# DLR-RM/curvature

Hardware: AMD Instinct MI355X
Metric: KFAC factor-build + invert + sample throughput (higher is better)
Workload: dtype f32

## Files before the change

### curvature_amd/csrc/invert.hip

```cpp
#include <type_traits>
#include "kernarg.h"
#include "mma64.h"
#include <hip/hip_ext.h>

#include <algorithm>
#include <chrono>
#include <cstdlib>
#include <mutex>
#include <vector>

namespace curv {

constexpr int INV_THREADS = MMA_THREADS;
constexpr int SQ_FLAGS = 32;
constexpr int SQ_FD = 0, SQ_FLC = 4, SQ_FLROW = 8, SQ_FT = 12;
constexpr int SQ_SPIN_LIMIT = 1 << 21;
#ifdef CURV_SQ_TRACE
__device__ long long g_sq_trace[256];
#define KT_BEGIN(slot) { if (threadIdx.x == 0 && k0 == 4 * (CURV_SQ_TRACE - 1)) atomicMax((unsigned long long*)&g_sq_trace[slot], (1ull << 62) - (unsigned long long)wall_clock64()); }
#define KT_END(slot) { if (threadIdx.x == 0 && k0 == 4 * (CURV_SQ_TRACE - 1)) atomicMax((unsigned long long*)&g_sq_trace[slot], (unsigned long long)wall_clock64()); }
#define SQT(slot) { if (threadIdx.x == 0 && f == 0 && stamp == CURV_SQ_TRACE) g_sq_trace[slot] = wall_clock64(); }
#define FIT(k) { if (threadIdx.x == 0 && trace_base >= 0) g_sq_trace[trace_base + (k)] = wall_clock64(); }
#else
#define SQT(slot)
#define FIT(k)
#define KT_BEGIN(slot) {}
#define KT_END(slot) {}
#endif
#ifdef CURV_SQ_TRACE
#define PQT(slot) { if (threadIdx.x == 0 && blockIdx.x == 0 && k0 == 4 * (CURV_SQ_TRACE - 1)) g_sq_trace[slot] = wall_clock64(); }
#else
#define PQT(slot)
#endif

struct InvDev {
  const float* F;
  float* L;
  double* W;
  double* X;
  int* info;
  int n, np, P;
  float sqrt_s, sqrt_n;
  int reverse;
  int f64_in;
  int r_minus;
  double* Xout;
  const double* R;
  double* Zm;
  double add64;
  float* C32;
  float* X32;
  float* S32;
  double pivot_min;
};
typedef __attribute__((address_space(1))) float gfloat;
__device__ __host__ __forceinline__ bool s_in_sweep(const InvDev& d) { return d.X32 == nullptr; }
__device__ __host__ __forceinline__ int s_kind(const InvDev& d) { return d.X32 != nullptr ? 0 : (d.Zm != nullptr ? 2 : 1); }

template <typename CountFn>
__device__ __forceinline__ bool locate(const InvDev* __restrict__ t, int nf, int bid, CountFn cnt, int& f,
                                       int& local) {
  const int lane = threadIdx.x & 63;
  int base = 0;
  for (int f0 = 0; f0 < nf; f0 += 64) {
    const int ff = f0 + lane;
    const int c = (ff < nf) ? cnt(t[ff]) : 0;
    int incl = c;
#pragma unroll
    for (int o = 1; o < 64; o <<= 1) {
      const int v = __shfl_up(incl, o, 64);
      if (lane >= o) incl += v;
    }
    const int total = __builtin_amdgcn_readfirstlane(__shfl(incl, 63, 64));
    if (bid < base + total) {
      const unsigned long long m = __ballot(bid < base + incl);
      const int l = __ffsll((long long)m) - 1;
      f = __builtin_amdgcn_readfirstlane(f0 + l);
      local = __builtin_amdgcn_readfirstlane(bid - (base + __shfl(incl - c, l, 64)));
      return true;
    }
    base += total;
  }
  return false;
}

__global__ void __launch_bounds__(INV_THREADS)
inv_prepare_kernel(const InvDev* __restrict__ t, int nf, int* __restrict__ flags) {
  int f, tile;
  if (!locate(t, nf, blockIdx.x, [](const InvDev& d) { return d.P * (d.P + 1) / 2; }, f, tile)) return;
  const InvDev& d = t[f];
  int bi = 0;
  while (tile > bi) { tile -= bi + 1; ++bi; }
  const int bj = tile;
  const int n = d.n, np = d.np, rev = d.reverse;
  const float ss = d.sqrt_s, sn = d.sqrt_n;
  const gfloat* F = (const gfloat*)d.F;
  gdouble* W = (gdouble*)d.W;
  if (bi == 0 && bj == 0 && threadIdx.x == 0) *d.info = 0;
  if (bi == 0 && bj == 0 && threadIdx.x < SQ_FLAGS) flags[(long long)f * SQ_FLAGS + threadIdx.x] = 0;
  if (d.Zm != nullptr) {
    const gdouble* Rg = (const gdouble*)d.R;
    gdouble* Z = (gdouble*)d.Zm;
    const int w0 = __builtin_amdgcn_readfirstlane(threadIdx.x >> 6), c0 = threadIdx.x & 63;
    const int jj = bj * NB + c0;
#pragma unroll 4
    for (int u = 0; u < 16; ++u) {
      const int i = bi * NB + w0 + 4 * u;
      Z[(long long)i * np + jj] = (i < n && jj <= i) ? Rg[(long long)i * n + jj] : 0.0;
    }
  }
  if (d.f64_in) {
    const gdouble* M = (const gdouble*)d.F;
    const int w0 = __builtin_amdgcn_readfirstlane(threadIdx.x >> 6), c0 = threadIdx.x & 63;
    const int jj = bj * NB + c0;
#pragma unroll 4
    for (int u = 0; u < 16; ++u) {
      const int i = bi * NB + w0 + 4 * u;
      double v;
      if (i < n && jj < n) {
        v = 0.5 * (M[(long long)i * n + jj] + M[(long long)jj * n + i]);
        if (i == jj) v += d.add64;
      } else {
        v = (i == jj) ? 1.0 : 0.0;
      }
      W[(long long)i * np + jj] = v;
    }
    return;
  }
  __shared__ float Tm[NB][NB + 1];
  const int w = __builtin_amdgcn_readfirstlane(threadIdx.x >> 6), c = threadIdx.x & 63;
  const int j = bj * NB + c, rj = rev ? n - 1 - j : j;
  const int mi = bi * NB + c, rmi = rev ? n - 1 - mi : mi;
  float fd[16], fm[16];
#pragma unroll
  for (int u = 0; u < 16; ++u) {
    const int r = w + 4 * u;
    const int i = bi * NB + r, ri = rev ? n - 1 - i : i;
    const int mj = bj * NB + r, rmj = rev ? n - 1 - mj : mj;
    fd[u] = (i < n && j < n) ? F[(long long)ri * n + rj] : 0.0f;
    fm[u] = (mi < n && mj < n) ? F[(long long)rmj * n + rmi] : 0.0f;
  }
#pragma unroll
  for (int u = 0; u < 16; ++u) Tm[w + 4 * u][c] = fm[u];
  __syncthreads();
#pragma unroll
  for (int u = 0; u < 16; ++u) {
    const int r = w + 4 * u;
    const int i = bi * NB + r;
    double v;
    if (i < n && j < n) {
      float a = __fmul_rn(ss, fd[u]);
      float b = __fmul_rn(ss, Tm[c][r]);
      if (i == j) { a = __fadd_rn(a, sn); b = __fadd_rn(b, sn); }
      v = (double)__fmul_rn(__fadd_rn(a, b), 0.5f);
    } else {
      v = (i == j) ? 1.0 : 0.0;
    }
    W[(long long)i * np + j] = v;
  }
}

__device__ __host__ __forceinline__ long long inner_tiles(int P, int k, int k0, int kend) {
  const int ke = kend < P ? kend : P;
  long long tr = 0;
  for (int j = k + 1; j < ke; ++j) tr += ke - j;
  const long long sr = (ke - k - 1 > 0) ? (long long)(ke - k - 1) * (k - k0 + 1) : 0;
  return tr + sr;
}
constexpr int SB = 4;
__device__ __host__ __forceinline__ long long outer_tiles(int P, int kend, int row0, bool s_part) {
  const long long r = P - row0;
  if (r <= 0) return 0;
  const long long nsb = (r + SB - 1) / SB, ncb = s_part ? (kend + SB - 1) / SB : 0;
  return (nsb * (nsb + 1) / 2 + nsb * ncb) * (SB * SB);
}
__device__ __host__ __forceinline__ long long strip_tiles(int P, int kend, int lo, int hi, bool s_part) {
  const int re = hi < P ? hi : P;
  long long n = 0;
  for (int j = lo; j < re; ++j) n += P - j;
  if (s_part && re > lo) n += (long long)(re - lo) * kend;
  return n;
}

__device__ __forceinline__ void store_sub(gdouble* C, int np, const f64x4 (&acc)[2][2], int wm, int wn, int lane,
                                          int mode) {
  store_acc(C, np, acc, wm, wn, lane, mode);
}

__device__ __forceinline__ void factor_invert_64(double* Ds, double* Is, int* bad, int pivot_base, double pivot_min, int trace_base = -1);
__device__ __forceinline__ void lds_sub_acc(double* s, const f64x4 (&acc)[2][2], int wm, int wn, int lane);

__global__ void __launch_bounds__(INV_THREADS)
inner_update_kernel(const InvDev* __restrict__ t, int nf, int k, int k0, int kend) {
  __shared__ double As[NB * LDA], Bs[NB * LDA];
  int f, local;
  if (!locate(t, nf, blockIdx.x, [k, k0, kend](const InvDev& d) { return (int)inner_tiles(d.P, k, k0, kend); }, f, local)) return;
  const InvDev& d = t[f];
  const int np = d.np, P = d.P, ke = kend < P ? kend : P;
  gdouble* W = (gdouble*)d.W;
  gdouble* X = (gdouble*)d.X;
  const int lane = threadIdx.x & 63, wave = threadIdx.x >> 6, wm = wave >> 1, wn = wave & 1;
  f64x4 acc[2][2] = {};
  int j = k + 1;
  bool trailing = false;
  for (; j < ke; ++j) {
    if (local < ke - j) { trailing = true; break; }
    local -= ke - j;
  }
  if (trailing) {
    const int i = j + local;
    load_block(W + (long long)i * NB * np + k * NB, np, As);
    if (i != j) load_block(W + (long long)j * NB * np + k * NB, np, Bs);
    __syncthreads();
    mma_64<true>(As, (i != j) ? Bs : As, wm, wn, lane, acc);
    if (i == j && j == k + 1) {
      __shared__ int bad;
      __syncthreads();
      if (threadIdx.x == 0) bad = 0;
      load_block(W + (long long)j * NB * np + j * NB, np, As);
      __syncthreads();
      {
        const int c16 = lane & 15, rq = lane >> 4;
#pragma unroll
        for (int m = 0; m < 2; ++m)
#pragma unroll
          for (int n = 0; n < 2; ++n)
#pragma unroll
            for (int q = 0; q < 4; ++q)
              As[(32 * wm + 16 * m + rq + 4 * q) * LDA + 32 * wn + 16 * n + c16] -= acc[m][n][q];
      }
      __syncthreads();
      factor_invert_64(As, Bs, &bad, j * NB, d.pivot_min);
      store_block(X + (long long)j * NB * np + j * NB, np, Bs);
      if (threadIdx.x == 0 && bad != 0) atomicCAS(d.info, 0, bad);
    } else {
      store_sub(W + (long long)i * NB * np + j * NB, np, acc, wm, wn, lane, 0);
    }
  } else {
    const int w = k - k0 + 1;
    const int a = local / w, jj = k0 + local - a * w;
    const int i = k + 1 + a;
// ... 102 lines not shown
    for (int q = 0; q < 4; ++q) {
      const double v = acc[0][0][q];
      const double out = o.mode == 0 ? old[q] - v : o.mode == 1 ? v : o.mode == 2 ? old[q] + v : -v;
      *(gdouble*)(base + (long long)(4 * q) * np * 8 + voff) = out;
    }
  }
}

template <int WV>
__device__ __forceinline__ void tile_product_k32(const TileJob& o, double* __restrict__ As, double* __restrict__ Bs) {
  if (!o.bt) tile_product_impl<WV, 2>(o, As, Bs);
  else if (o.same) tile_product_impl<WV, 1>(o, As, Bs);
  else tile_product_impl<WV, 0>(o, As, Bs);
}

template <int WV>
__device__ __forceinline__ void outer_update_body(const InvDev* __restrict__ t, int nf, int k0, int kend, int lo, int hi,
                                                  int strip, int n_items, double* __restrict__ As, double* __restrict__ Bs) {
  bool trailing;
  int i, j, f, local;
  if (strip == 1) {
    if (!locate(t, nf, blockIdx.x, [kend, lo, hi](const InvDev& d) { return (int)strip_tiles(d.P, kend, lo, hi, s_in_sweep(d)); }, f, local))
      return;
    const int P = t[f].P, re = hi < P ? hi : P;
    trailing = false;
    j = lo;
    for (; j < re; ++j) {
      if (local < P - j) { trailing = true; break; }
      local -= P - j;
    }
    if (trailing) {
      i = j + local;
    } else {
      const int a = local / kend;
      i = lo + a; j = local - a * kend;
    }
  } else {
    const int row0 = lo;
    int item;
    {
      const int bid = blockIdx.x, xcd = bid & 7, jj = bid >> 3;
      item = ((jj / (SB * SB)) * 8 + xcd) * (SB * SB) + (jj % (SB * SB));
    }
    if (item >= n_items) return;
    if (!locate(t, nf, item, [kend, row0](const InvDev& d) {
          return (int)(outer_tiles(d.P, kend, row0, s_in_sweep(d)) - outer_tiles(d.P, kend, row0, false)); }, f, local)) return;
    const int r = t[f].P - row0;
    const int s2 = local / (SB * SB), in = local % (SB * SB);
    const int di = in / SB, dj = in - di * SB;
    const int ncb = (kend + SB - 1) / SB;
    const int a = s2 / ncb, cb = s2 - a * ncb;
    const int ri = a * SB + di; j = cb * SB + dj;
    if (ri >= r || j >= kend) return;
    trailing = false; i = row0 + ri;
  }
  const InvDev& d = t[f];
  const int np = d.np;
  const gdouble* W = (const gdouble*)d.W;
  gdouble* X = (gdouble*)d.X;
  TileJob o;
  o.np = np;
  o.bt = trailing;
  o.same = trailing && i == j;
  o.a0 = (const gbyte*)(W + (long long)i * NB * np);
  gdouble* Sx = d.Zm != nullptr ? (gdouble*)d.Zm : X;
  o.b0 = trailing ? (const gbyte*)(W + (long long)j * NB * np) : (const gbyte*)(Sx + j * NB);
  o.ke0 = (trailing ? k0 : (j > k0 ? j : k0)) * NB;
  o.ke1 = kend * NB;
  o.C = trailing ? (gdouble*)d.W + (long long)i * NB * np + j * NB : Sx + (long long)i * NB * np + j * NB;
  o.mode = trailing ? 0 : (d.Zm != nullptr ? 0 : (j >= k0 ? 1 : 2));
  tile_product_k32<WV>(o, As, Bs);
}
__global__ void __launch_bounds__(INV_THREADS, 3)
outer_update_kernel(const InvDev* __restrict__ t, int nf, int k0, int kend, int lo, int hi, int strip, int n_items) {
  __shared__ double As[NB * OPA], Bs[NB * OPA > OKS * LDA ? NB * OPA : OKS * LDA];
  outer_update_body<2>(t, nf, k0, kend, lo, hi, strip, n_items, As, Bs);
}
typedef __attribute__((address_space(3))) void lds_void;
typedef __attribute__((address_space(3))) char lds_char;
typedef double f64x2 __attribute__((ext_vector_type(2)));
namespace fard {
constexpr int ROW_B = 128, TILE_B = NB * ROW_B, KS = 16;
}
__global__ void __launch_bounds__(INV_THREADS, 4)
outer_update_dma_kernel(const InvDev* __restrict__ t, int nf, int k0, int kend, int row0, int n_items) {
  using namespace fard;
  __shared__ __attribute__((aligned(1024))) char smem[4 * TILE_B];
  lds_char* lds = (lds_char*)smem;
  int item;
  {
    const int bid = blockIdx.x, xcd = bid & 7, jj = bid >> 3;
    item = ((jj / (SB * SB)) * 8 + xcd) * (SB * SB) + (jj % (SB * SB));
  }
  if (item >= n_items) return;
  int f, local;
  if (!locate(t, nf, item, [kend, row0](const InvDev& d) { return (int)outer_tiles(d.P, kend, row0, false); }, f, local)) return;
  const InvDev& d = t[f];
  int i, j;
  {
    const int r = d.P - row0;
    const int sb = local / (SB * SB), in = local - sb * (SB * SB);
    const int di = in / SB, dj = in - di * SB;
    int a = 0, tl = sb;
    while (tl > a) { tl -= a + 1; ++a; }
    const int ri = a * SB + di, rj = tl * SB + dj;
    if (ri >= r || rj > ri) return;
    i = row0 + ri; j = row0 + rj;
  }
  const int np = d.np;
  const int tid = threadIdx.x, lane = tid & 63;
  const int wave = __builtin_amdgcn_readfirstlane(tid >> 6), wm = wave >> 1, wn = wave & 1;
  const int r16 = lane & 15, kq = lane >> 4;
  const bool same = i == j;
  const unsigned panel_b = (unsigned)((long long)NB * np * 8);
  const __amdgpu_buffer_rsrc_t rs_a =
      __builtin_amdgcn_make_buffer_rsrc((void*)(d.W + (long long)i * NB * np), 0, panel_b, 0x00020000);
  const __amdgpu_buffer_rsrc_t rs_b =
      __builtin_amdgcn_make_buffer_rsrc((void*)(d.W + (long long)j * NB * np), 0, panel_b, 0x00020000);
  const int drow = 8 * wave + (lane >> 3);
  const int voff = (drow * np) * 8 + (((lane & 7) ^ ((drow >> 1) & 7)) << 4);
  const int half_b = 32 * np * 8;
  auto issue = [&](int ke, unsigned buf) {
    const int kb = ke * 8;
    __builtin_amdgcn_raw_ptr_buffer_load_lds(rs_a, (lds_void*)(lds + buf + wave * 1024), 16, voff, kb, 0, 0);
    __builtin_amdgcn_raw_ptr_buffer_load_lds(rs_a, (lds_void*)(lds + buf + (wave + 4) * 1024), 16, voff, half_b + kb, 0, 0);
    if (!same) {
      __builtin_amdgcn_raw_ptr_buffer_load_lds(rs_b, (lds_void*)(lds + 2 * TILE_B + buf + wave * 1024), 16, voff, kb, 0, 0);
      __builtin_amdgcn_raw_ptr_buffer_load_lds(rs_b, (lds_void*)(lds + 2 * TILE_B + buf + (wave + 4) * 1024), 16, voff, half_b + kb, 0, 0);
    }
  };
  unsigned addr_a[2], addr_b[2];
#pragma unroll
  for (int m = 0; m < 2; ++m) {
    const int ra = 32 * wm + 16 * m + r16, rb = 32 * wn + 16 * m + r16;
    addr_a[m] = ra * ROW_B + ((kq ^ ((ra >> 1) & 7)) << 4);
    addr_b[m] = (same ? 0 : 2 * TILE_B) + rb * ROW_B + ((kq ^ ((rb >> 1) & 7)) << 4);
  }
  f64x4 acc[2][2] = {};
  const int ke0 = k0 * NB, n_st = (kend - k0) * NB / KS;
  issue(ke0, 0);
  for (int st = 0; st < n_st; ++st) {
    __builtin_amdgcn_s_waitcnt(0x0f70);
    __syncthreads();
    const unsigned buf = (st & 1) * TILE_B;
    if (st + 1 < n_st) issue(ke0 + KS * (st + 1), TILE_B - buf);
    f64x2 av[2][2], bv[2][2];
#pragma unroll
    for (int h = 0; h < 2; ++h)
#pragma unroll
      for (int m = 0; m < 2; ++m) {
        av[m][h] = *reinterpret_cast<const __attribute__((address_space(3))) f64x2*>(lds + buf + (addr_a[m] ^ (h << 6)));
        bv[m][h] = *reinterpret_cast<const __attribute__((address_space(3))) f64x2*>(lds + buf + (addr_b[m] ^ (h << 6)));
      }
#pragma unroll
    for (int h = 0; h < 2; ++h)
#pragma unroll
      for (int dd = 0; dd < 2; ++dd)
#pragma unroll
        for (int m = 0; m < 2; ++m)
#pragma unroll
          for (int n = 0; n < 2; ++n) acc[m][n] = __builtin_amdgcn_mfma_f64_16x16x4f64(av[m][h][dd], bv[n][h][dd], acc[m][n], 0, 0, 0);
  }
  store_acc((gdouble*)d.W + (long long)i * NB * np + j * NB, np, acc, wm, wn, lane, 0);
}

__global__ void __launch_bounds__(1024)
outer_update_wide_kernel(const InvDev* __restrict__ t, int nf, int k0, int kend, int lo, int hi, int strip, int n_items) {
  __shared__ double As[NB * OPA], Bs[NB * OPA > OKS * LDA ? NB * OPA : OKS * LDA];
  KT_BEGIN(252)
  outer_update_body<4>(t, nf, k0, kend, lo, hi, strip, n_items, As, Bs);
  KT_END(253)
}

__device__ __forceinline__ double readlane_f64(double v, int src_lane) {
  const int lo = __builtin_amdgcn_readlane(__double2loint(v), src_lane);
  const int hi = __builtin_amdgcn_readlane(__double2hiint(v), src_lane);
  return __hiloint2double(hi, lo);
}

template <bool BT>
__device__ __forceinline__ void mma16(const double* Ap, int lda, const double* Bp, int ldb, int lane, f64x4& acc) {
  const int r16 = lane & 15, kq = lane >> 4;
#pragma unroll
  for (int ks = 0; ks < 4; ++ks) {
    const int kk = 4 * ks + kq;
    const double a = Ap[r16 * lda + kk];
    const double b = BT ? Bp[r16 * ldb + kk] : Bp[kk * ldb + r16];
    acc = __builtin_amdgcn_mfma_f64_16x16x4f64(a, b, acc, 0, 0, 0);
  }
}

__device__ __forceinline__ double rsqrt_pos(double x) {
  double y = __builtin_amdgcn_rsq(x);
  const double hx = 0.5 * x;
  y = y * fma(-hx * y, y, 1.5);
  y = y * fma(-hx * y, y, 1.5);
  return y;
}

__device__ __forceinline__ double rcp_pos(double x) {
  const double y = __builtin_amdgcn_rcp(x);
  const double e = fma(-x, y, 1.0);
  return fma(y, fma(e, e, e), y);
}

__device__ __forceinline__ void factor_invert_64(double* Ds, double* Is, int* bad, int pivot_base, double pivot_min, int trace_base) {
  (void)trace_base;
  __shared__ double Sc[4][16 * 17];
  __shared__ double dinv_s[NB];
  const int tid = threadIdx.x, lane = tid & 63, wave = tid >> 6;
  const int r16 = lane & 15, kq = lane >> 4;
  auto diag_inverse = [&](int b) {
    if (lane < 16) {
      const double* Lb = Ds + 16 * b * LDA + 16 * b;
      double x[16], sum[16], col[16], dv[16];
#pragma unroll
      for (int r = 0; r < 16; ++r) { sum[r] = 0.0; col[r] = r > 0 ? Lb[r * LDA] : 0.0; dv[r] = dinv_s[16 * b + r]; }
#pragma unroll
      for (int q = 0; q < 16; ++q) {
        x[q] = ((q == lane ? 1.0 : 0.0) - sum[q]) * dv[q];
        double nxt[16];
#pragma unroll
        for (int r = q + 2; r < 16; ++r) nxt[r] = Lb[r * LDA + q + 1];
#pragma unroll
        for (int r = q + 1; r < 16; ++r) sum[r] += col[r] * x[q];
#pragma unroll
        for (int r = q + 2; r < 16; ++r) col[r] = nxt[r];
      }
#pragma unroll
      for (int r = 0; r < 16; ++r) Is[(16 * b + r) * LDA + 16 * b + lane] = x[r];
    }
  };
  auto wave_sync = [&]() {
    __builtin_amdgcn_fence(__ATOMIC_RELEASE, "wavefront");
    __builtin_amdgcn_wave_barrier();
    __builtin_amdgcn_fence(__ATOMIC_ACQUIRE, "wavefront");
  };
  auto block_sum = [&](int i, int b, int k_lo, int k_hi, f64x4& acc) {
    for (int kk = k_lo; kk < k_hi; ++kk)
      mma16<false>(Ds + 16 * i * LDA + 16 * kk, LDA, Is + 16 * kk * LDA + 16 * b, LDA, lane, acc);
  };
  auto finish_block = [&](int i, int b, const f64x4& acc) {
#pragma unroll
    for (int r = 0; r < 4; ++r) Sc[wave][(kq + 4 * r) * 17 + r16] = acc[r];
// ... 464 lines not shown
  int cf = c, kf = kb;
  fetch(cf, kf, rt0); next(cf, kf);
  if (cf >= 0) { fetch(cf, kf, rt1); next(cf, kf); }
  if (cf >= 0) { fetch(cf, kf, rt2); next(cf, kf); }
  f64x4 acc[4] = {};
  PQT(241)
  [[maybe_unused]] int pq_n = 0;
  auto step = [&](double (&rt)[16]) __attribute__((always_inline)) {
    __syncthreads();
#pragma unroll
    for (int u = 0; u < 16; ++u) Ts[((tid >> 6) + 4 * u) * LDA + (tid & 63)] = rt[u];
    __syncthreads();
    if (cf >= 0) { fetch(cf, kf, rt); next(cf, kf); }
#pragma unroll
    for (int ks = 0; ks < NB / 4; ++ks) {
      const int k = 4 * ks + kq;
      const double a = below ? Own[r16 * PQ_PITCH + 64 * kb + k] : Ts[(16 * wave + r16) * LDA + k];
      const double b = below ? Ts[(16 * wave + r16) * LDA + k] : Own[(64 * kb + k) * 17 + r16];
      acc[ks & 3] = __builtin_amdgcn_mfma_f64_16x16x4f64(a, b, acc[ks & 3], 0, 0, 0);
    }
    if (kb == c) {
      const int wm = below ? q : wave, wn = below ? wave : q;
      const int c16 = lane & 15, rq = lane >> 4;
      gbyte* base = below ? (gbyte*)d.W + (((long long)i * NB) * np + (long long)(k0 + c) * NB) * 8
                          : (gbyte*)d.X + (((long long)(k0 + c) * NB) * np + (long long)j * NB) * 8;
      const unsigned voff = (unsigned)(((long long)(16 * wm + rq) * np + 16 * wn + c16) * 8);
      gbyte* base32 = (below && d.C32 != nullptr) ? (gbyte*)d.C32 + (((long long)i * NB) * np + (long long)(k0 + c) * NB) * 4 : nullptr;
      const unsigned voff32 = (unsigned)(((long long)(16 * wm + rq) * np + 16 * wn + c16) * 4);
#pragma unroll
      for (int qq = 0; qq < 4; ++qq) {
        const double v = (acc[0][qq] + acc[1][qq]) + (acc[2][qq] + acc[3][qq]);
        *(gdouble*)(base + (long long)(4 * qq) * np * 8 + voff) = below ? v : -v;
        if (below && base32 != nullptr) *(gfloat*)(base32 + (long long)(4 * qq) * np * 4 + voff32) = (float)v;
      }
#pragma unroll
      for (int u = 0; u < 4; ++u) acc[u] = f64x4{0.0, 0.0, 0.0, 0.0};
    }
    next(c, kb);
    PQT(242 + pq_n)
    ++pq_n;
  };
  while (c >= 0) {
    step(rt0);
    if (c < 0) break;
    step(rt1);
    if (c < 0) break;
    step(rt2);
  }
}
__global__ void __launch_bounds__(INV_THREADS)
panel_product_quarter_kernel(const InvDev* __restrict__ t, int nf, int k0, int kend) {
  __shared__ double Own[PQ_OWN], Ts[NB * LDA];
  const int job = (blockIdx.x >> 5) * 8 + (blockIdx.x & 7), q = (blockIdx.x >> 3) & 3;
  int f, local;
  KT_BEGIN(236)
  if (!locate(t, nf, job, [k0, kend](const InvDev& d) { return panel_jobs(d.P, s_kind(d), k0, kend); }, f, local)) return;
  const InvDev& d = t[f];
  const int nb = (kend < d.P ? kend : d.P) - k0;
  const int n_below = d.P > kend ? d.P - kend : 0;
  if (local < n_below) panel_quarter_body<true>(d, k0, nb, kend + local, 0, q, Own, Ts);
  else panel_quarter_body<false>(d, k0, nb, 0, local - n_below, q, Own, Ts);
  KT_END(237)
}
__global__ void __launch_bounds__(INV_THREADS, 3)
panel_product_kernel(const InvDev* __restrict__ t, int nf, int k0, int kend) {
  __shared__ double As[NB * OPA], Bs[NB * OPA > OKS * LDA ? NB * OPA : OKS * LDA];
  panel_product_body<2>(t, nf, k0, kend, As, Bs);
}
__global__ void __launch_bounds__(1024)
panel_product_wide_kernel(const InvDev* __restrict__ t, int nf, int k0, int kend) {
  __shared__ double As[NB * OPA], Bs[NB * OPA > OKS * LDA ? NB * OPA : OKS * LDA];
  panel_product_body<4>(t, nf, k0, kend, As, Bs);
}

constexpr int SKS = 32;
constexpr int SPA = SKS + 1;
constexpr int SPB = NB + 32;
struct Tile32 {
  const gbyte* a;
  const gbyte* b;
  gfloat* out;
  int np, ke0, ke1;
  bool a64, b64, accumulate, negate;
};
__device__ __forceinline__ void tile32(const Tile32& o, float* __restrict__ As, float* __restrict__ Bs) {
  const int np = o.np;
  const int tid = threadIdx.x, lane = tid & 63, wave = tid >> 6, wm = wave >> 1, wn = wave & 1;
  const int l32 = lane & 31, h = lane >> 5;
  const long long a_off = (long long)(tid >> 3) * np + 4 * (tid & 7), a_step = 32ll * np;
  const long long b_off = (long long)(tid >> 4) * np + 4 * (tid & 15), b_step = 16ll * np;
  typedef const __attribute__((address_space(1))) f32x4 gf4;
  typedef const __attribute__((address_space(1))) f64x4 gd4;
  f32x4 ra[2], rb[2];
  auto fetch = [&](int ke) __attribute__((always_inline)) {
    if (o.a64) {
#pragma unroll
      for (int u = 0; u < 2; ++u) {
        const f64x4 v = *(gd4*)(o.a + (a_off + u * a_step + ke) * 8);
        ra[u] = f32x4{(float)v[0], (float)v[1], (float)v[2], (float)v[3]};
      }
    } else {
#pragma unroll
      for (int u = 0; u < 2; ++u) ra[u] = *(gf4*)(o.a + (a_off + u * a_step + ke) * 4);
    }
    if (o.b64) {
#pragma unroll
      for (int u = 0; u < 2; ++u) {
        const f64x4 v = *(gd4*)(o.b + (b_off + u * b_step + (long long)ke * np) * 8);
        rb[u] = f32x4{(float)v[0], (float)v[1], (float)v[2], (float)v[3]};
      }
    } else {
#pragma unroll
      for (int u = 0; u < 2; ++u) rb[u] = *(gf4*)(o.b + (b_off + u * b_step + (long long)ke * np) * 4);
    }
  };
  f32x16 acc = {0};
  fetch(o.ke0);
  for (int ke = o.ke0; ke < o.ke1; ke += SKS) {
#pragma unroll
    for (int u = 0; u < 2; ++u)
#pragma unroll
      for (int e = 0; e < 4; ++e) {
        As[((tid >> 3) + 32 * u) * SPA + 4 * (tid & 7) + e] = ra[u][e];
        Bs[((tid >> 4) + 16 * u) * SPB + 4 * (tid & 15) + e] = rb[u][e];
      }
    __syncthreads();
    if (ke + SKS < o.ke1) fetch(ke + SKS);
#pragma unroll
    for (int kk = 0; kk < SKS; kk += 2) {
      const float av = As[(32 * wm + l32) * SPA + kk + h];
      const float bv = Bs[(kk + h) * SPB + 32 * wn + l32];
      acc = __builtin_amdgcn_mfma_f32_32x32x2f32(av, bv, acc, 0, 0, 0);
    }
    __syncthreads();
  }
  gbyte* base = (gbyte*)(o.out + (long long)(32 * wm + 4 * h) * np + 32 * wn + l32);
  if (!o.accumulate) {
#pragma unroll
    for (int reg = 0; reg < 16; ++reg)
      *(gfloat*)(base + (long long)((reg & 3) + 8 * (reg >> 2)) * np * 4) = o.negate ? -acc[reg] : acc[reg];
  } else {
    float old[16];
#pragma unroll
    for (int reg = 0; reg < 16; ++reg) old[reg] = *(const gfloat*)(base + (long long)((reg & 3) + 8 * (reg >> 2)) * np * 4);
#pragma unroll
    for (int reg = 0; reg < 16; ++reg) *(gfloat*)(base + (long long)((reg & 3) + 8 * (reg >> 2)) * np * 4) = old[reg] + acc[reg];
  }
}
__device__ __host__ __forceinline__ long long supd_tiles(int P, int kind, int kend) {
  if (kind != 0 || P <= kend) return 0;
  const long long nsb = (P - kend + SB - 1) / SB, ncb = (kend + SB - 1) / SB;
  return nsb * ncb * (SB * SB);
}
__global__ void __launch_bounds__(INV_THREADS, 3)
supd32_kernel(const InvDev* __restrict__ t, int nf, int k0, int kend, int n_items) {
  __shared__ float As[NB * SPA], Bs[SKS * SPB];
  int item;
  {
    const int bid = blockIdx.x, xcd = bid & 7, jj = bid >> 3;
    item = ((jj / (SB * SB)) * 8 + xcd) * (SB * SB) + (jj % (SB * SB));
  }
  if (item >= n_items) return;
  int f, local;
  if (!locate(t, nf, item, [kend](const InvDev& d) { return (int)supd_tiles(d.P, s_kind(d), kend); }, f, local)) return;
  const InvDev& d = t[f];
  const int np = d.np, r = d.P - kend;
  const int ncb = (kend + SB - 1) / SB;
  const int sb = local / (SB * SB), in = local - sb * (SB * SB);
  const int a = sb / ncb, cb = sb - a * ncb;
  const int ri = a * SB + in / SB, j = cb * SB + in % SB;
  if (ri >= r || j >= kend) return;
  const int i = kend + ri;
  const bool own = j >= k0;
  Tile32 o;
  o.np = np;
  o.a = (const gbyte*)((const gfloat*)d.C32 + (long long)i * NB * np);
  o.a64 = false;
  o.b = own ? (const gbyte*)((const gdouble*)d.X + j * NB) : (const gbyte*)((const gfloat*)d.X32 + j * NB);
  o.b64 = own;
  o.ke0 = (own ? j : k0) * NB;
  o.ke1 = kend * NB;
  o.out = (gfloat*)d.S32 + (long long)i * NB * np + j * NB;
  o.accumulate = !own;
  o.negate = false;
  tile32(o, As, Bs);
}
__device__ __host__ __forceinline__ long long xrow_tiles(int P, int kind, int k0, int kend) {
  if (kind != 0 || P <= k0) return 0;
  return (long long)((kend < P ? kend : P) - k0) * k0;
}
__global__ void __launch_bounds__(INV_THREADS, 3)
xrows32_kernel(const InvDev* __restrict__ t, int nf, int k0, int kend) {
  __shared__ float As[NB * SPA], Bs[SKS * SPB];
  int f, local;
  if (!locate(t, nf, blockIdx.x, [k0, kend](const InvDev& d) { return (int)xrow_tiles(d.P, s_kind(d), k0, kend); }, f, local)) return;
  const InvDev& d = t[f];
  const int np = d.np, nb = (kend < d.P ? kend : d.P) - k0;
  const int j = local / nb, c = nb - 1 - (local - j * nb);
  Tile32 o;
  o.np = np;
  o.a = (const gbyte*)((const gdouble*)d.X + (long long)(k0 + c) * NB * np);
  o.a64 = true;
  o.b = (const gbyte*)((const gfloat*)d.S32 + j * NB);
  o.b64 = false;
  o.ke0 = k0 * NB;
  o.ke1 = (k0 + c + 1) * NB;
  o.out = (gfloat*)d.X32 + (long long)(k0 + c) * NB * np + j * NB;
  o.accumulate = false;
  o.negate = true;
  tile32(o, As, Bs);
}

__global__ void __launch_bounds__(INV_THREADS)
inv_finalize_kernel(const InvDev* __restrict__ t, int nf, int sq) {
  __shared__ float tile[NB][NB + 1];
  int f, local;
  if (!locate(t, nf, blockIdx.x, [](const InvDev& d) { return d.P * d.P; }, f, local)) return;
  const InvDev& d = t[f];
  const int n = d.n, np = d.np, q = d.P;
  const int ti = local / q, tj = local - ti * q;
  const gdouble* X = (const gdouble*)d.X;
  const gfloat* X32 = (const gfloat*)d.X32;
  gfloat* L = (gfloat*)d.L;
  const int w = __builtin_amdgcn_readfirstlane(threadIdx.x >> 6), c = threadIdx.x & 63;
  if (!d.reverse) {
    gdouble* Xo = (gdouble*)d.Xout;
    const gdouble* S = d.Zm != nullptr ? (const gdouble*)d.Zm : X;
#pragma unroll 4
    for (int u = 0; u < 16; ++u) {
      const int i = ti * NB + w + 4 * u, j = tj * NB + c;
      if (i < n && j < n) {
        double v = (j <= i) ? S[(long long)i * np + j] : 0.0;
        if (d.r_minus && j <= i) v = ((const gdouble*)d.R)[(long long)i * n + j] - v;
        Xo[(long long)i * n + j] = v;
      }
    }
    return;
  }
  if (tj > ti) {
#pragma unroll 4
    for (int u = 0; u < 16; ++u) {
      const int i = ti * NB + w + 4 * u, j = tj * NB + c;
      if (i < n && j < n) L[(long long)i * n + j] = 0.0f;
    }
    return;
  }
  double xv[16];
  const int i_l = ti * NB + c;
#pragma unroll
  for (int u = 0; u < 16; ++u) {
    const int j = tj * NB + w + 4 * u;
    const int rs = n - 1 - j, cs = n - 1 - i_l;
    const bool live = i_l < n && j < n && j <= i_l;
    if (X32 == nullptr || rs / sq == cs / sq) xv[u] = live ? X[(long long)rs * np + cs] : 0.0;
    else xv[u] = live ? (double)X32[(long long)rs * np + cs] : 0.0;
  }
#pragma unroll
  for (int u = 0; u < 16; ++u) tile[w + 4 * u][c] = (float)xv[u];
  __syncthreads();
#pragma unroll
  for (int u = 0; u < 16; ++u) {
    const int i = ti * NB + w + 4 * u, j = tj * NB + c;
    if (i < n && j < n) L[(long long)i * n + j] = tile[c][w + 4 * u];
  }
}

constexpr int INV_UPLOAD_CHUNK = 28;
static_assert(sizeof(InvDev) * INV_UPLOAD_CHUNK <= 3840, "a new InvDev field needs a hole in the row or a smaller chunk");

static size_t inv_table_bytes(int n) { return align_up((size_t)std::max(n, 1) * sizeof(InvDev), 256); }
static size_t inv_flags_bytes(int n) { return align_up((size_t)std::max(n, 1) * SQ_FLAGS * sizeof(int), 256); }

struct SideStream {
  hipStream_t stream = nullptr;
  hipEvent_t ev_main[2] = {nullptr, nullptr};
  hipEvent_t ev_side[2] = {nullptr, nullptr};
  hipEvent_t ev_tail = nullptr;
};
struct StreamSet {
  SideStream side[2];
  hipStream_t aux = nullptr;
  hipStream_t masked = nullptr;
  hipEvent_t ev_fork = nullptr, ev_join = nullptr, ev_join2 = nullptr;
  hipEvent_t ev_chain[2] = {nullptr, nullptr};
};
static std::mutex g_masked_mutex;
static std::vector<std::pair<int, hipStream_t>> g_masked_streams;
static void destroy_masked_streams() {
  std::lock_guard<std::mutex> lock(g_masked_mutex);
  for (auto& e : g_masked_streams) {
    if (hipSetDevice(e.first) == hipSuccess) {
      (void)hipStreamSynchronize(e.second);
      (void)hipStreamDestroy(e.second);
    }
  }
  g_masked_streams.clear();
}

static int stream_set(StreamSet** out) {
  static thread_local std::vector<std::pair<int, StreamSet>> cache;
  int dev = 0;
  CURV_HIP_CHECK(hipGetDevice(&dev));
  for (auto& e : cache) if (e.first == dev) { *out = &e.second; return CURV_OK; }
  StreamSet s;
  int prio_low = 0, prio_high = 0;
  CURV_HIP_CHECK(hipDeviceGetStreamPriorityRange(&prio_low, &prio_high));
  CURV_HIP_CHECK(hipEventCreateWithFlags(&s.ev_fork, hipEventDisableTiming));
  CURV_HIP_CHECK(hipEventCreateWithFlags(&s.ev_join, hipEventDisableTiming));
  CURV_HIP_CHECK(hipEventCreateWithFlags(&s.ev_join2, hipEventDisableTiming));
  for (int g = 0; g < 2; ++g) CURV_HIP_CHECK(hipEventCreateWithFlags(&s.ev_chain[g], hipEventDisableTiming));
  auto wide_stream = [&](hipStream_t* out) -> int {
    static const int free_cus = getenv("CURV_FREE_CUS") ? atoi(getenv("CURV_FREE_CUS")) : 32;
    hipDeviceProp_t prop;
    int dev_id = 0;
    CURV_HIP_CHECK(hipGetDevice(&dev_id));
    CURV_HIP_CHECK(hipGetDeviceProperties(&prop, dev_id));
    const int n_cu = prop.multiProcessorCount;
    if (free_cus > 0 && 2 * free_cus <= n_cu) {
      std::vector<uint32_t> mask((size_t)cdiv(n_cu, 32), 0u);
      for (int c = 0; c < n_cu - free_cus; ++c) mask[c >> 5] |= 1u << (c & 31);
      if (hipExtStreamCreateWithCUMask(out, (uint32_t)mask.size(), mask.data()) == hipSuccess) {
        std::lock_guard<std::mutex> lock(g_masked_mutex);
        if (g_masked_streams.empty()) atexit(destroy_masked_streams);
        g_masked_streams.emplace_back(dev_id, *out);
        return CURV_OK;
      }
      (void)hipGetLastError();
    }
    CURV_HIP_CHECK(hipStreamCreateWithPriority(out, hipStreamNonBlocking, prio_low));
    return CURV_OK;
  };
  CURV_HIP_CHECK(hipStreamCreateWithPriority(&s.aux, hipStreamNonBlocking, prio_high));
  CURV_HIP_CHECK(hipStreamCreateWithFlags(&s.masked, hipStreamNonBlocking));
  for (int g = 0; g < 2; ++g) {
    { const int rc = wide_stream(&s.side[g].stream); if (rc != CURV_OK) return rc; }
    for (int i = 0; i < 2; ++i) {
      CURV_HIP_CHECK(hipEventCreateWithFlags(&s.side[g].ev_main[i], hipEventDisableTiming));
      CURV_HIP_CHECK(hipEventCreateWithFlags(&s.side[g].ev_side[i], hipEventDisableTiming));
    }
    CURV_HIP_CHECK(hipEventCreateWithFlags(&s.side[g].ev_tail, hipEventDisableTiming));
  }
  cache.emplace_back(dev, s);
  *out = &cache.back().second;
  return CURV_OK;
}

int curv_internal_side_stream(hipStream_t* out) {
  StreamSet* ss = nullptr;
  const int rc = stream_set(&ss);
  if (rc != CURV_OK) return rc;
  *out = ss->masked;
  return CURV_OK;
}

}

using namespace curv;

#ifdef CURV_SQ_TRACE
extern "C" int curv_debug_sq_trace_reset() {
  long long zeros[256] = {0};
  return hipMemcpyToSymbol(HIP_SYMBOL(curv::g_sq_trace), zeros, sizeof(zeros)) == hipSuccess ? 0 : 1;
}
extern "C" int curv_debug_sq_trace(long long* out) {
  return hipMemcpyFromSymbol(out, HIP_SYMBOL(curv::g_sq_trace), 256 * sizeof(long long)) == hipSuccess ? 0 : 1;
}
#endif

extern "C" int curv_init_streams(void) {
  StreamSet* ss = nullptr;
  return stream_set(&ss);
}

extern "C" size_t curv_chol_inv_workspace_bytes(const curv_inv_desc* descs, int n_factors) {
  size_t total = 2 * inv_table_bytes(n_factors) + 2 * inv_flags_bytes(n_factors);
  for (int i = 0; i < n_factors; ++i) {
    if (descs[i].n <= 0) return 0;
    const size_t np = (size_t)cdiv(descs[i].n, NB) * NB;
    total += 2 * np * np * sizeof(double) + 3 * np * np * sizeof(float);
  }
  return total;
}

static int sweep_nbo(bool latency_bound) { return latency_bound ? 4 : 6; }
struct GroupSweep {
  hipStream_t stream;
  SideStream* side;
  const std::vector<InvDev>* tabp;
  InvDev* table;
  int* flags;
  bool latency_bound;
  int n_factors = 0, Pmax = 0, NBO = 4, k0 = 0, panel = 0;
  long long fin_tiles = 0, quarter_prod = 0;
  bool use_square = false, far_pending = false, inv_pending = false, capturing = false;

  GroupSweep(hipStream_t st, SideStream* sd, const std::vector<InvDev>& tab, InvDev* tb, int* fl, bool lb)
      : stream(st), side(sd), tabp(&tab), table(tb), flags(fl), latency_bound(lb) {}
  bool done() const { return k0 >= Pmax; }
  int panels() const { return cdiv(Pmax, NBO); }

  int begin() {
    const std::vector<InvDev>& tab = *tabp;
    n_factors = (int)tab.size();
    hipStreamCaptureStatus cap = hipStreamCaptureStatusNone;
    CURV_HIP_CHECK(hipStreamIsCapturing(stream, &cap));
    capturing = cap != hipStreamCaptureStatusNone;
    long long prep_tiles = 0;
    for (const InvDev& d : tab) {
      Pmax = std::max(Pmax, d.P);
      prep_tiles += (long long)d.P * (d.P + 1) / 2;
      fin_tiles += (long long)d.P * d.P;
    }
    const int rcu = upload_table<INV_UPLOAD_CHUNK>(stream, table, tab.data(), n_factors);
    if (rcu != CURV_OK) return rcu;
    hipLaunchKernelGGL(inv_prepare_kernel, dim3((unsigned)prep_tiles), dim3(INV_THREADS), 0, stream, table, n_factors, flags);
    CURV_LAUNCH_CHECK();
    NBO = sweep_nbo(latency_bound);
    return CURV_OK;
  }

  int panel_step() {
    const std::vector<InvDev>& tab = *tabp;
    constexpr long long WIDE_NEAR = 512, WIDE_PROD = 256;
    constexpr long long QUARTER_PROD = 512;
    quarter_prod = latency_bound ? QUARTER_PROD : 0;
    use_square = latency_bound;
    const int kend = k0 + NBO, row0 = kend + NBO;
    long long prod_tiles = 0;
    if (use_square) {
      long long sq_wgs = 0;
      for (const InvDev& d : tab)
        if (d.P > k0) sq_wgs += std::min(kend, d.P) - k0;
      hipLaunchKernelGGL(chol_square_kernel, dim3((unsigned)sq_wgs), dim3(INV_THREADS), 0, stream, table, n_factors, k0, kend,
                         flags, panel + 1);
      CURV_LAUNCH_CHECK();
    }
    for (int k = k0; !use_square && k < std::min(kend, Pmax); ++k) {
      long long diag_tiles = 0, panel_tiles = 0, upd_tiles = 0;
      for (const InvDev& d : tab) {
        if (d.P > k) { ++diag_tiles; panel_tiles += std::min(kend, d.P) - k0 - 1; }
        upd_tiles += inner_tiles(d.P, k, k0, kend);
      }
      if (k == k0) {
        hipLaunchKernelGGL(chol_diag_kernel, dim3((unsigned)diag_tiles), dim3(INV_THREADS), 0, stream, table, n_factors, k);
        CURV_LAUNCH_CHECK();
      }
      if (panel_tiles > 0) {
        hipLaunchKernelGGL(chol_panel_kernel, dim3((unsigned)panel_tiles), dim3(INV_THREADS), 0, stream, table, n_factors, k, k0, kend);
        CURV_LAUNCH_CHECK();
      }
      if (upd_tiles > 0) {
        hipLaunchKernelGGL(inner_update_kernel, dim3((unsigned)upd_tiles), dim3(INV_THREADS), 0, stream, table, n_factors, k, k0, kend);
        CURV_LAUNCH_CHECK();
      }
    }
    auto launch_product = [&](hipStream_t st, long long jobs, hipEvent_t done) -> int {
      const InvDev* tb = table;
      if (jobs <= quarter_prod)
        hipExtLaunchKernelGGL(panel_product_quarter_kernel, dim3((unsigned)(cdivll(jobs, 8) * 32)), dim3(INV_THREADS), 0, st,
                              nullptr, done, 0, tb, n_factors, k0, kend);
      else if (jobs <= WIDE_PROD)
        hipExtLaunchKernelGGL(panel_product_wide_kernel, dim3((unsigned)jobs), dim3(1024), 0, st, nullptr, done, 0, tb, n_factors,
                              k0, kend);
      else
        hipExtLaunchKernelGGL(panel_product_kernel, dim3((unsigned)jobs), dim3(INV_THREADS), 0, st, nullptr, done, 0, tb,
                              n_factors, k0, kend);
      CURV_LAUNCH_CHECK();
      return CURV_OK;
    };
    long long inv_jobs = 0, inv_tiles = 0;
    for (const InvDev& d : tab) {
      prod_tiles += panel_jobs(d.P, s_kind(d), k0, kend);
      inv_jobs += xrow_tiles(d.P, s_kind(d), k0, kend);
      inv_tiles += supd_tiles(d.P, s_kind(d), kend);
    }
    bool fork_recorded = false;
    if (prod_tiles > 0) {
      fork_recorded = !capturing;
      const int rc = launch_product(stream, prod_tiles, fork_recorded ? side->ev_main[panel & 1] : nullptr);
      if (rc != CURV_OK) return rc;
    }
    long long near_tiles = 0, far_tiles = 0;
    for (const InvDev& d : tab) {
      near_tiles += strip_tiles(d.P, kend, kend, row0, s_in_sweep(d));
      far_tiles += outer_tiles(d.P, kend, row0, s_in_sweep(d));
    }
    hipStream_t inv_st = side->stream;
    const bool inv_work = inv_jobs > 0 || inv_tiles > 0;
    const bool side_work = far_tiles > 0 || inv_work;
    if (side_work) {
      if (!fork_recorded) CURV_HIP_CHECK(hipEventRecord(side->ev_main[panel & 1], stream));
      CURV_HIP_CHECK(hipStreamWaitEvent(side->stream, side->ev_main[panel & 1], 0));
    }
    if (near_tiles > 0) {
      if (far_pending) {
        CURV_HIP_CHECK(hipStreamWaitEvent(stream, side->ev_side[(panel + 1) & 1], 0));
      }
      far_pending = false;
      if (near_tiles <= WIDE_NEAR)
        hipLaunchKernelGGL(outer_update_wide_kernel, dim3((unsigned)near_tiles), dim3(1024), 0, stream, table, n_factors,
                           k0, kend, kend, row0, 1, (int)near_tiles);
      else
        hipLaunchKernelGGL(outer_update_kernel, dim3((unsigned)near_tiles), dim3(INV_THREADS), 0, stream, table, n_factors, k0,
                           kend, kend, row0, 1, (int)near_tiles);
      CURV_LAUNCH_CHECK();
    }
    if (far_tiles > 0) {
      const bool ride = !capturing;
      const InvDev* tb = table;
      long long trail = 0;
      for (const InvDev& d : tab) trail += outer_tiles(d.P, kend, row0, false);
      const long long s_tiles = far_tiles - trail;
      if (trail > 0) {
        const long long g1 = cdivll(trail, 8 * SB * SB) * 8 * SB * SB;
        hipExtLaunchKernelGGL(outer_update_dma_kernel, dim3((unsigned)g1), dim3(INV_THREADS), 0, side->stream, nullptr,
                              (ride && s_tiles == 0) ? side->ev_side[panel & 1] : nullptr, 0, tb, n_factors, k0, kend, row0, (int)trail);
        CURV_LAUNCH_CHECK();
      }
      if (s_tiles > 0) {
        const long long g2 = cdivll(s_tiles, 8 * SB * SB) * 8 * SB * SB;
        hipExtLaunchKernelGGL(outer_update_kernel, dim3((unsigned)g2), dim3(INV_THREADS), 0, side->stream, nullptr,
                              ride ? side->ev_side[panel & 1] : nullptr, 0, tb, n_factors, k0, kend, row0, 0, 2, (int)s_tiles);
        CURV_LAUNCH_CHECK();
      }
      if (!ride) CURV_HIP_CHECK(hipEventRecord(side->ev_side[panel & 1], side->stream));
      far_pending = true;
    }
    if (inv_jobs > 0) {
      hipLaunchKernelGGL(xrows32_kernel, dim3((unsigned)inv_jobs), dim3(INV_THREADS), 0, inv_st, table, n_factors, k0, kend);
      CURV_LAUNCH_CHECK();
      inv_pending = true;
    }
    if (inv_tiles > 0) {
      const long long grid = cdivll(inv_tiles, 8 * SB * SB) * 8 * SB * SB;
      hipLaunchKernelGGL(supd32_kernel, dim3((unsigned)grid), dim3(INV_THREADS), 0, inv_st, table, n_factors, k0, kend,
                         (int)inv_tiles);
      CURV_LAUNCH_CHECK();
      inv_pending = true;
    }
    k0 += NBO;
    ++panel;
    return CURV_OK;
  }

  int end(hipEvent_t chain_done = nullptr) {
    if (chain_done != nullptr) CURV_HIP_CHECK(hipEventRecord(chain_done, stream));
    if (far_pending) CURV_HIP_CHECK(hipStreamWaitEvent(stream, side->ev_side[(panel + 1) & 1], 0));
    if (inv_pending) {
      CURV_HIP_CHECK(hipEventRecord(side->ev_tail, side->stream));
      CURV_HIP_CHECK(hipStreamWaitEvent(stream, side->ev_tail, 0));
    }
    hipLaunchKernelGGL(inv_finalize_kernel, dim3((unsigned)fin_tiles), dim3(INV_THREADS), 0, stream, table, n_factors, NBO * NB);
    CURV_LAUNCH_CHECK();
    return CURV_OK;
  }
};

static int chol_sweep_group(hipStream_t stream, SideStream* side, const std::vector<InvDev>& tab, InvDev* table, int* flags,
                            bool latency_bound, hipEvent_t chain_done = nullptr) {
  GroupSweep g(stream, side, tab, table, flags, latency_bound);
  int rc = g.begin();
  while (rc == CURV_OK && !g.done()) rc = g.panel_step();
  return rc == CURV_OK ? g.end(chain_done) : rc;
}

constexpr int SPLIT_P = 16;

struct EarlyStatus { int* host; const int* dev; size_t bytes; hipEvent_t ev; };

static int await_verdict(const EarlyStatus* early) {
  if (early != nullptr) CURV_HIP_CHECK(hipEventSynchronize(early->ev));
  return CURV_OK;
}

static int chol_sweep(hipStream_t stream, std::vector<InvDev>& tab, void* workspace, size_t workspace_bytes,
                      const char* who, const EarlyStatus* early = nullptr) {
  const int n_factors = (int)tab.size();
  static const int latency_max = getenv("CURV_LATENCY_MAX") ? atoi(getenv("CURV_LATENCY_MAX")) : 64;
  bool any_rhs = false;
  for (const InvDev& d : tab) any_rhs = any_rhs || d.R != nullptr;
  const bool latency_bound = n_factors <= latency_max && !any_rhs;
  size_t need = 2 * inv_table_bytes(n_factors) + 2 * inv_flags_bytes(n_factors);
  for (const InvDev& d : tab)
    need += (d.R != nullptr ? 3 : 2) * (size_t)d.np * d.np * sizeof(double) + (d.reverse ? 3 * (size_t)d.np * d.np * sizeof(float) : 0);
  if (workspace == nullptr || workspace_bytes < need) {
    set_error("%s: workspace too small (%zu < %zu bytes)", who, workspace_bytes, need);
    return CURV_ERR_WORKSPACE;
  }
  char* p = reinterpret_cast<char*>(workspace) + 2 * inv_table_bytes(n_factors);
  int* flags0 = reinterpret_cast<int*>(p);
  int* flags1 = reinterpret_cast<int*>(p + inv_flags_bytes(n_factors));
  p += 2 * inv_flags_bytes(n_factors);
  std::vector<InvDev> big, small;
  int Pmax = 0;
  for (const InvDev& d : tab) Pmax = std::max(Pmax, d.P);
  const int split = std::max(SPLIT_P, Pmax / 2);
  for (InvDev& d : tab) {
    d.W = reinterpret_cast<double*>(p); p += (size_t)d.np * d.np * sizeof(double);
// ... 166 lines not shown
```

Measured before the change: 4195.

## Fuse damped-factor preparation into first far update and emit L directly

```diff
diff --git a/curvature_amd/csrc/invert.hip b/curvature_amd/csrc/invert.hip
--- a/curvature_amd/csrc/invert.hip
+++ b/curvature_amd/csrc/invert.hip
@@ -84,13 +84,32 @@
   return false;
 }
 
+__device__ __host__ __forceinline__ long long outer_tiles(int P, int kend, int row0, bool s_part);
+__device__ __host__ __forceinline__ int far_first_col(const InvDev& d, int nbo) {
+  return (d.reverse && outer_tiles(d.P, nbo, 2 * nbo, false) > 0) ? 2 * nbo : d.P;
+}
+__device__ __host__ __forceinline__ int prepare_tiles(const InvDev& d, int nbo) {
+  const int c = far_first_col(d, nbo);
+  return c * (c + 1) / 2 + (d.P - c) * c;
+}
+__device__ __forceinline__ float damped_element(float fd, float fm, float ss, float sn, int i, int j, int n) {
+  if (i < n && j < n) {
+    float a = __fmul_rn(ss, fd);
+    float b = __fmul_rn(ss, fm);
+    if (i == j) { a = __fadd_rn(a, sn); b = __fadd_rn(b, sn); }
+    return __fmul_rn(__fadd_rn(a, b), 0.5f);
+  }
+  return (i == j) ? 1.0f : 0.0f;
+}
+
 __global__ void __launch_bounds__(INV_THREADS)
-inv_prepare_kernel(const InvDev* __restrict__ t, int nf, int* __restrict__ flags) {
+inv_prepare_kernel(const InvDev* __restrict__ t, int nf, int* __restrict__ flags, int nbo) {
   int f, tile;
-  if (!locate(t, nf, blockIdx.x, [](const InvDev& d) { return d.P * (d.P + 1) / 2; }, f, tile)) return;
+  if (!locate(t, nf, blockIdx.x, [nbo](const InvDev& d) { return prepare_tiles(d, nbo); }, f, tile)) return;
   const InvDev& d = t[f];
+  const int cmax = far_first_col(d, nbo);
   int bi = 0;
-  while (tile > bi) { tile -= bi + 1; ++bi; }
+  for (int w = 1; tile >= w; w = (bi + 1 < cmax ? bi + 1 : cmax)) { tile -= w; ++bi; }
   const int bj = tile;
   const int n = d.n, np = d.np, rev = d.reverse;
   const float ss = d.sqrt_s, sn = d.sqrt_n;
@@ -147,16 +166,7 @@
   for (int u = 0; u < 16; ++u) {
     const int r = w + 4 * u;
     const int i = bi * NB + r;
-    double v;
-    if (i < n && j < n) {
-      float a = __fmul_rn(ss, fd[u]);
-      float b = __fmul_rn(ss, Tm[c][r]);
-      if (i == j) { a = __fadd_rn(a, sn); b = __fadd_rn(b, sn); }
-      v = (double)__fmul_rn(__fadd_rn(a, b), 0.5f);
-    } else {
-      v = (i == j) ? 1.0 : 0.0;
-    }
-    W[(long long)i * np + j] = v;
+    W[(long long)i * np + j] = (double)damped_element(fd[u], Tm[c][r], ss, sn, i, j, n);
   }
 }
 
@@ -425,6 +435,7 @@
 namespace fard {
 constexpr int ROW_B = 128, TILE_B = NB * ROW_B, KS = 16;
 }
+template <bool FIRST>
 __global__ void __launch_bounds__(INV_THREADS, 4)
 outer_update_dma_kernel(const InvDev* __restrict__ t, int nf, int k0, int kend, int row0, int n_items) {
   using namespace fard;
@@ -479,6 +490,23 @@
     addr_a[m] = ra * ROW_B + ((kq ^ ((ra >> 1) & 7)) << 4);
     addr_b[m] = (same ? 0 : 2 * TILE_B) + rb * ROW_B + ((kq ^ ((rb >> 1) & 7)) << 4);
   }
+  const bool fresh = FIRST && j >= far_first_col(d, kend - k0);
+  const int fw = wave, fc = lane;
+  [[maybe_unused]] float fd[16], fm[16];
+  if constexpr (FIRST) {
+    if (fresh) {
+      const int n = d.n;
+      const gfloat* F = (const gfloat*)d.F;
+      const int cj = j * NB + fc, mi = i * NB + fc;
+#pragma unroll
+      for (int u = 0; u < 16; ++u) {
+        const int r = fw + 4 * u;
+        const int ri = i * NB + r, mj = j * NB + r;
+        fd[u] = (ri < n && cj < n) ? F[(long long)(n - 1 - ri) * n + (n - 1 - cj)] : 0.0f;
+        fm[u] = (mi < n && mj < n) ? F[(long long)(n - 1 - mj) * n + (n - 1 - mi)] : 0.0f;
+      }
+    }
+  }
   f64x4 acc[2][2] = {};
   const int ke0 = k0 * NB, n_st = (kend - k0) * NB / KS;
   issue(ke0, 0);
@@ -503,6 +531,42 @@
         for (int m = 0; m < 2; ++m)
 #pragma unroll
           for (int n = 0; n < 2; ++n) acc[m][n] = __builtin_amdgcn_mfma_f64_16x16x4f64(av[m][h][dd], bv[n][h][dd], acc[m][n], 0, 0, 0);
+  }
+  if constexpr (FIRST) {
+    if (fresh) {
+      constexpr int TP = NB + 1;
+      static_assert(NB * TP * sizeof(float) <= 4 * TILE_B, "the transposition tile lives in the stage buffers");
+      float* Tm = (float*)smem;
+      const float ss = d.sqrt_s, sn = d.sqrt_n;
+      const int n = d.n;
+      __syncthreads();
+#pragma unroll
+      for (int u = 0; u < 16; ++u) Tm[(fw + 4 * u) * TP + fc] = fm[u];
+      __syncthreads();
+      float v[16];
+#pragma unroll
+      for (int u = 0; u < 16; ++u) {
+        const int r = fw + 4 * u;
+        v[u] = damped_element(fd[u], Tm[fc * TP + r], ss, sn, i * NB + r, j * NB + fc, n);
+      }
+      __syncthreads();
+#pragma unroll
+      for (int u = 0; u < 16; ++u) Tm[(fw + 4 * u) * TP + fc] = v[u];
+      __syncthreads();
+      const int c16 = lane & 15, rq = lane >> 4;
+      const unsigned voff_c = (unsigned)(((long long)(32 * wm + rq) * np + 32 * wn + c16) * 8);
+      gbyte* base = (gbyte*)((gdouble*)d.W + (long long)i * NB * np + j * NB);
+#pragma unroll
+      for (int m = 0; m < 2; ++m)
+#pragma unroll
+        for (int nn = 0; nn < 2; ++nn)
+#pragma unroll
+          for (int q = 0; q < 4; ++q) {
+            const double old = (double)Tm[(32 * wm + 16 * m + rq + 4 * q) * TP + 32 * wn + 16 * nn + c16];
+            *(gdouble*)(base + ((long long)(16 * m + 4 * q) * np + 16 * nn) * 8 + voff_c) = old - acc[m][nn][q];
+          }
+      return;
+    }
   }
   store_acc((gdouble*)d.W + (long long)i * NB * np + j * NB, np, acc, wm, wn, lane, 0);
 }
@@ -1133,8 +1197,21 @@
   gfloat* out;
   int np, ke0, ke1;
   bool a64, b64, accumulate, negate;
+  gfloat* L = nullptr;
+  int n = 0, r0 = 0, c0 = 0;
 };
-__device__ __forceinline__ void tile32(const Tile32& o, float* __restrict__ As, float* __restrict__ Bs) {
+constexpr int LTP = NB + 1;
+__device__ __forceinline__ void emit_L_tile(const float* __restrict__ Lt, gfloat* __restrict__ L, int n, int r0, int c0) {
+  const int w = __builtin_amdgcn_readfirstlane(threadIdx.x >> 6), rl = threadIdx.x & 63;
+  const int r = r0 + rl;
+#pragma unroll
+  for (int u = 0; u < 16; ++u) {
+    const int cl = w + 4 * u, c = c0 + cl;
+    if (r < n && c < n) L[(long long)(n - 1 - c) * n + (n - 1 - r)] = Lt[cl * LTP + rl];
+  }
+}
+template <bool EMIT_L = false>
+__device__ __forceinline__ void tile32(const Tile32& o, float* __restrict__ As, float* __restrict__ Bs, float* Lt = nullptr) {
   const int np = o.np;
   const int tid = threadIdx.x, lane = tid & 63, wave = tid >> 6, wm = wave >> 1, wn = wave & 1;
   const int l32 = lane & 31, h = lane >> 5;
@@ -1188,8 +1265,15 @@
   gbyte* base = (gbyte*)(o.out + (long long)(32 * wm + 4 * h) * np + 32 * wn + l32);
   if (!o.accumulate) {
 #pragma unroll
-    for (int reg = 0; reg < 16; ++reg)
-      *(gfloat*)(base + (long long)((reg & 3) + 8 * (reg >> 2)) * np * 4) = o.negate ? -acc[reg] : acc[reg];
+    for (int reg = 0; reg < 16; ++reg) {
+      const float v = o.negate ? -acc[reg] : acc[reg];
+      *(gfloat*)(base + (long long)((reg & 3) + 8 * (reg >> 2)) * np * 4) = v;
+      if constexpr (EMIT_L) Lt[(32 * wn + l32) * LTP + 32 * wm + 4 * h + (reg & 3) + 8 * (reg >> 2)] = v;
+    }
+    if constexpr (EMIT_L) {
+      __syncthreads();
+      emit_L_tile(Lt, o.L, o.n, o.r0, o.c0);
+    }
   } else {
     float old[16];
 #pragma unroll
@@ -1242,7 +1326,10 @@
 }
 __global__ void __launch_bounds__(INV_THREADS, 3)
 xrows32_kernel(const InvDev* __restrict__ t, int nf, int k0, int kend) {
-  __shared__ float As[NB * SPA], Bs[SKS * SPB];
+  static_assert(NB * SPA + SKS * SPB >= NB * LTP, "the operand tiles hold a transposed 64 x 64 tile");
+  __shared__ __attribute__((aligned(16))) float sm[NB * SPA + SKS * SPB];
+  float* As = sm;
+  float* Bs = sm + NB * SPA;
   int f, local;
   if (!locate(t, nf, blockIdx.x, [k0, kend](const InvDev& d) { return (int)xrow_tiles(d.P, s_kind(d), k0, kend); }, f, local)) return;
   const InvDev& d = t[f];
@@ -1259,21 +1346,65 @@
   o.out = (gfloat*)d.X32 + (long long)(k0 + c) * NB * np + j * NB;
   o.accumulate = false;
   o.negate = true;
-  tile32(o, As, Bs);
-}
-
+  o.L = (gfloat*)d.L; o.n = d.n; o.r0 = (k0 + c) * NB; o.c0 = j * NB;
+  tile32<true>(o, As, Bs, sm);
+}
+
+constexpr int ZS = 4;
+__device__ __host__ __forceinline__ int zero_strips(int P) {
+  const int m = P - 1, q = m / ZS, r = m - q * ZS;
+  return ZS * (q * (q + 1) / 2) + r * (q + 1);
+}
+__device__ __host__ __forceinline__ int finalize_tiles(const InvDev& d, int nbo) {
+  if (!d.reverse) return d.P * d.P;
+  const int q = d.P / nbo, r = d.P - q * nbo;
+  return zero_strips(d.P) + q * (nbo * (nbo + 1) / 2) + r * (r + 1) / 2;
+}
 __global__ void __launch_bounds__(INV_THREADS)
 inv_finalize_kernel(const InvDev* __restrict__ t, int nf, int sq) {
-  __shared__ float tile[NB][NB + 1];
+  __shared__ float tile[NB * LTP];
   int f, local;
-  if (!locate(t, nf, blockIdx.x, [](const InvDev& d) { return d.P * d.P; }, f, local)) return;
+  const int nbo = sq / NB;
+  if (!locate(t, nf, blockIdx.x, [nbo](const InvDev& d) { return finalize_tiles(d, nbo); }, f, local)) return;
   const InvDev& d = t[f];
   const int n = d.n, np = d.np, q = d.P;
-  const int ti = local / q, tj = local - ti * q;
   const gdouble* X = (const gdouble*)d.X;
-  const gfloat* X32 = (const gfloat*)d.X32;
   gfloat* L = (gfloat*)d.L;
   const int w = __builtin_amdgcn_readfirstlane(threadIdx.x >> 6), c = threadIdx.x & 63;
+  if (d.reverse) {
+    const int n_zero = zero_strips(q);
+    if (local < n_zero) {
+      int bj = 1;
+      for (int s = 1; local >= s; s = (bj + ZS - 1) / ZS) { local -= s; ++bj; }
+      const int bi0 = local * ZS, nt = (bj - bi0 < ZS ? bj - bi0 : ZS);
+#pragma unroll 4
+      for (int u = 0; u < 16; ++u) {
+        const int cc = bj * NB + w + 4 * u;
+        for (int s = 0; s < nt; ++s) {
+          const int r = (bi0 + s) * NB + c;
+          if (r < n && cc < n) L[(long long)(n - 1 - cc) * n + (n - 1 - r)] = 0.0f;
+        }
+      }
+      return;
+    }
+    local -= n_zero;
+    const int per = nbo * (nbo + 1) / 2, s = local / per;
+    int a = 0, b = local - s * per;
+    while (b > a) { b -= a + 1; ++a; }
+    const int r0 = (s * nbo + a) * NB, c0 = (s * nbo + b) * NB;
+    double xv[16];
+#pragma unroll
+    for (int u = 0; u < 16; ++u) {
+      const int r = r0 + w + 4 * u, cc = c0 + c;
+      xv[u] = (r < n && cc <= r) ? X[(long long)r * np + cc] : 0.0;
+    }
+#pragma unroll
+    for (int u = 0; u < 16; ++u) tile[c * LTP + w + 4 * u] = (float)xv[u];
+    __syncthreads();
+    emit_L_tile(tile, L, n, r0, c0);
+    return;
+  }
+  const int ti = local / q, tj = local - ti * q;
   if (!d.reverse) {
     gdouble* Xo = (gdouble*)d.Xout;
     const gdouble* S = d.Zm != nullptr ? (const gdouble*)d.Zm : X;
@@ -1287,32 +1418,6 @@
       }
     }
     return;
-  }
-  if (tj > ti) {
-#pragma unroll 4
-    for (int u = 0; u < 16; ++u) {
-      const int i = ti * NB + w + 4 * u, j = tj * NB + c;
-      if (i < n && j < n) L[(long long)i * n + j] = 0.0f;
-    }
-    return;
-  }
-  double xv[16];
-  const int i_l = ti * NB + c;
-#pragma unroll
-  for (int u = 0; u < 16; ++u) {
-    const int j = tj * NB + w + 4 * u;
-    const int rs = n - 1 - j, cs = n - 1 - i_l;
-    const bool live = i_l < n && j < n && j <= i_l;
-    if (X32 == nullptr || rs / sq == cs / sq) xv[u] = live ? X[(long long)rs * np + cs] : 0.0;
-    else xv[u] = live ? (double)X32[(long long)rs * np + cs] : 0.0;
-  }
-#pragma unroll
-  for (int u = 0; u < 16; ++u) tile[w + 4 * u][c] = (float)xv[u];
-  __syncthreads();
-#pragma unroll
-  for (int u = 0; u < 16; ++u) {
-    const int i = ti * NB + w + 4 * u, j = tj * NB + c;
-    if (i < n && j < n) L[(long long)i * n + j] = tile[c][w + 4 * u];
   }
 }
 
@@ -1444,6 +1549,7 @@
   int n_factors = 0, Pmax = 0, NBO = 4, k0 = 0, panel = 0;
   long long fin_tiles = 0, quarter_prod = 0;
   bool use_square = false, far_pending = false, inv_pending = false, capturing = false;
+  bool far_first = false;
 
   GroupSweep(hipStream_t st, SideStream* sd, const std::vector<InvDev>& tab, InvDev* tb, int* fl, bool lb)
       : stream(st), side(sd), tabp(&tab), table(tb), flags(fl), latency_bound(lb) {}
@@ -1456,17 +1562,19 @@
     hipStreamCaptureStatus cap = hipStreamCaptureStatusNone;
     CURV_HIP_CHECK(hipStreamIsCapturing(stream, &cap));
     capturing = cap != hipStreamCaptureStatusNone;
+    NBO = sweep_nbo(latency_bound);
     long long prep_tiles = 0;
     for (const InvDev& d : tab) {
       Pmax = std::max(Pmax, d.P);
-      prep_tiles += (long long)d.P * (d.P + 1) / 2;
-      fin_tiles += (long long)d.P * d.P;
+      prep_tiles += prepare_tiles(d, NBO);
+      fin_tiles += finalize_tiles(d, NBO);
+      far_first = far_first || far_first_col(d, NBO) < d.P;
     }
     const int rcu = upload_table<INV_UPLOAD_CHUNK>(stream, table, tab.data(), n_factors);
     if (rcu != CURV_OK) return rcu;
-    hipLaunchKernelGGL(inv_prepare_kernel, dim3((unsigned)prep_tiles), dim3(INV_THREADS), 0, stream, table, n_factors, flags);
+    hipLaunchKernelGGL(inv_prepare_kernel, dim3((unsigned)prep_tiles), dim3(INV_THREADS), 0, stream, table, n_factors, flags,
+                       NBO);
     CURV_LAUNCH_CHECK();
-    NBO = sweep_nbo(latency_bound);
     return CURV_OK;
   }
 
@@ -1564,7 +1672,8 @@
       const long long s_tiles = far_tiles - trail;
       if (trail > 0) {
         const long long g1 = cdivll(trail, 8 * SB * SB) * 8 * SB * SB;
-        hipExtLaunchKernelGGL(outer_update_dma_kernel, dim3((unsigned)g1), dim3(INV_THREADS), 0, side->stream, nullptr,
+        auto far_kernel = (k0 == 0 && far_first) ? outer_update_dma_kernel<true> : outer_update_dma_kernel<false>;
+        hipExtLaunchKernelGGL(far_kernel, dim3((unsigned)g1), dim3(INV_THREADS), 0, side->stream, nullptr,
                               (ride && s_tiles == 0) ? side->ev_side[panel & 1] : nullptr, 0, tb, n_factors, k0, kend, row0, (int)trail);
         CURV_LAUNCH_CHECK();
       }
```

Result: no change. 4158 (-0.9%).
